# rajashree-srikanth/drone-sim-python

Measured on AMD Instinct MI355X. Metric: trajectory-optimisations/sec (6-seg poly, 50 wpts), higher is better.
Workload: dtype f64 residual/gradient + f32 MFMA J^T J

## Files before the change

drone-sim-python_amd/csrc/fit_basis.cpp:

```cpp
#include <cmath>
#include <cstring>

#include "fit_plan.h"

namespace {

double arr(int k, int n) {
  double a = 1;
  for (int i = n; i > n - k; --i) a *= i;
  return a;
}

struct Dense {
  int r, c;
  std::vector<double> a;
  Dense(int r_, int c_) : r(r_), c(c_), a((size_t)r_ * c_, 0.0) {}
  double &operator()(int i, int j) { return a[(size_t)i * c + j]; }
  double operator()(int i, int j) const { return a[(size_t)i * c + j]; }
};

Dense matmul(const Dense &A, const Dense &B, bool tA = false) {
  const int m = tA ? A.c : A.r, k = tA ? A.r : A.c, n = B.c;
  Dense C(m, n);
  for (int i = 0; i < m; ++i)
// ... 30 lines not shown
  for (int c = 0; c < n; ++c) {
    int piv = c;
    for (int r = c + 1; r < n; ++r)
      if (std::fabs(A(r, c)) > std::fabs(A(piv, c))) piv = r;
    if (A(piv, c) == 0.0) return false;
    for (int j = 0; j < n; ++j) {
      std::swap(A(c, j), A(piv, j));
      std::swap(I(c, j), I(piv, j));
    }
    const double ip = 1.0 / A(c, c);
    for (int j = 0; j < n; ++j) { A(c, j) *= ip; I(c, j) *= ip; }
    for (int r = 0; r < n; ++r) {
      if (r == c) continue;
      const double f = A(r, c);
      for (int j = 0; j < n; ++j) { A(r, j) -= f * A(c, j); I(r, j) -= f * I(c, j); }
    }
  }
  A = I;
  return true;
}

}

int fit_basis_build(d2d_fit_plan *pl) {
  const int S = pl->S, K = pl->K, nz = 8 * S, nk = 4 * (S + 1), nq = 4 * S;
  const double T = pl->duration / S;
  pl->T = T;
  pl->nq = nq;
  std::vector<int> seg(K);
  std::vector<double> tau(K);
  {
    std::vector<double> ends(S);
    double acc = 0;
    for (int s = 0; s < S; ++s) { acc += T; ends[s] = acc; }
    for (int k = 0; k < K; ++k) {
      const double step = pl->duration / (K - 1);
      const double t = (k == K - 1) ? pl->duration : k * step;
      int s = S - 1;
      for (int j = 0; j < S; ++j)
        if (ends[j] > t) { s = j; break; }
      seg[k] = s;
      tau[k] = t - s * T;
    }
  }
  pl->seg = seg;
  pl->tau = tau;
  std::vector<Dense> Phi;
  for (int d = 0; d < 3; ++d) {
    Dense P(K, nz);
    for (int k = 0; k < K; ++k)
      for (int p = d; p < 8; ++p) P(k, 8 * seg[k] + p) = arr(d, p) * std::pow(tau[k], p - d);
    Phi.push_back(P);
  }
  Dense M3(4, 4), M4(4, 4);
  for (int i = 0; i < 4; ++i) {
    for (int j = i; j < 4; ++j) M3(i, j) = arr(i, j) * std::pow(T, j - i);
    for (int j = 0; j < 4; ++j) M4(i, j) = arr(i, j + 4) * std::pow(T, j - i + 4);
  }
  if (!invert(M4)) { d2d_set_error("fit_basis_build: singular Hermite block"); return D2D_EINVAL; }
  Dense H(8, 8);
  for (int i = 0; i < 4; ++i) H(i, i) = 1.0 / arr(i, i);
  {
    Dense M1i(4, 4);
    for (int i = 0; i < 4; ++i) M1i(i, i) = 1.0 / arr(i, i);
    Dense t = matmul(matmul(M4, M3), M1i);
    for (int i = 0; i < 4; ++i)
      for (int j = 0; j < 4; ++j) { H(4 + i, j) = -t(i, j); H(4 + i, 4 + j) = M4(i, j); }
// ... 165 lines not shown
    A(k, k) = 1.0;
    for (int p = k; p < 8; ++p) {
      double c = 1.0;
      for (int i = 0; i < k; ++i) c = c * (p - i) / (i + 1);
      A(4 + k, p) = c;
    }
  }
  if (!invert(A)) { d2d_set_error("fit_basis_knots: singular Hermite block"); return D2D_EINVAL; }
  kn.Hb64.assign((size_t)K * KN_HB_STRIDE, 0.0);
  kn.Hb32.assign((size_t)K * 32, 0.f);
  for (int k = 0; k < K; ++k) {
    const double x = pl->tau[k] / T;
    const int s = pl->seg[k];
    for (int d = 0; d < 3; ++d)
      for (int m = 0; m < 8; ++m) {
        double v = 0.0;
        for (int p = d; p < 8; ++p) v += arr(d, p) * std::pow(x, p - d) * A(p, m);
        v /= std::pow(T, d);
        kn.Hb64[(size_t)k * KN_HB_STRIDE + 4 * m + d] = v;
        const bool fixed = (s == 0 && m < 2) || (s == S - 1 && m >= 4 && m < 6);
        kn.Hb32[(size_t)k * 32 + 4 * m + d] = fixed ? 0.f : (float)v;
      }
  }
  for (int s = 0; s <= S; ++s) kn.k0[s] = s < S ? pl->seg_k0[s] : K;
  for (int s = 0; s < S; ++s)
    if (pl->seg_Ks[s] == 0) kn.k0[s] = s + 1 < S ? pl->seg_k0[s + 1] : K;
  for (int s = S + 1; s <= D2D_FIT_MAX_S; ++s) kn.k0[s] = K;
  kn.Wseg.assign((size_t)S * 4 * 64, 0.f);
  for (int s = 0; s < S; ++s)
    for (int r = 0; r < 4; ++r)
      for (int l = 0; l < 64; ++l) {
        const int R = 4 * (l >> 4) + r, C = l & 15;
        const int aR = (R >> 2) & 1, aC = (C >> 2) & 1, mR = 4 * (R >> 3) + (R & 3), mC = 4 * (C >> 3) + (C & 3);
        if (aR != aC) continue;
        double v = 0.0;
        for (int k = kn.k0[s]; k < kn.k0[s + 1]; ++k) v += (double)kn.Hb32[(size_t)k * 32 + 4 * mR] * (double)kn.Hb32[(size_t)k * 32 + 4 * mC];
        kn.Wseg[((size_t)s * 4 + r) * 64 + l] = (float)v;
      }
  Dense L(nq, nq), Bm(nq, nq), Bi(nq, nq), Mu(nq, nq);
  for (int i = 0; i < nq; ++i)
    for (int j = 0; j < nq; ++j) L(i, j) = pl->Lw[(size_t)i * nq + j];
  std::vector<double> ds(nq);
  for (int i = 0; i < nq; ++i) ds[i] = dsc[freec[i] % 4];
  for (int j = 0; j < nq; ++j)
    for (int i = 0; i < nq; ++i) Bm(j, i) = L(i, j) / ds[i];
  Bi = Bm;
  if (!invert(Bi)) { d2d_set_error("fit_basis_knots: singular map"); return D2D_EINVAL; }
  Mu = matmul(Bm, Bm, true);
  Dense Mi = Mu;
  if (!invert(Mi)) { d2d_set_error("fit_basis_knots: singular metric"); return D2D_EINVAL; }
// ... 52 lines not shown
```

drone-sim-python_amd/csrc/fit_knot.hip:

```cpp
#include <cstdlib>
#include <vector>

#include "fit_phases.h"
#include "fit_plan.h"

#define KN_WPB_MAX 8
#define KN_LDS_BYTES (160 * 1024)
#define KN_N 48
#define KN_NE 56
#define KN_WV_KNOT 10
#define KN_US 10
#define KN_GTOL_SCALE 0.1
#define KN_SEG_MAX 11
#define KN_IMG_LS (KN_N + 4)

namespace {

#define LAUNDER_S(v) do { (v) = __builtin_amdgcn_readfirstlane(v); asm volatile("" : "+s"(v)); } while (0)

struct KnotGeom {
  int K, S, smax;
  int k0[D2D_FIT_MAX_S + 2];
};

struct KnotLds {
  int Hb64, Hb32, Wseg, Md32, Mi32, Mr32, Msc, wave0, wave_stride;
  int wv, sp, sfull, gfull, park, big, cf, cfp;
  int total;
};

inline int align16(int v) { return (v + 15) & ~15; }

KnotLds knot_lds_layout(int K, int wpb) {
  KnotLds L;
  int o = 0;
  L.Hb64 = o; o = align16(o + K * KN_HB_STRIDE * 8);
// ... 142 lines not shown
    for (int j = 0; j < 3; ++j) {
      const int s = s0 + j;
      int kb = kg.k0[s];
      n[j] = kg.k0[s + 1] - kg.k0[s];
      LAUNDER_S(kb); LAUNDER_S(n[j]);
#pragma unroll
      for (int i = 0; i < SEGMAX; ++i) {
        const int kk = kb + (i < n[j] ? i : (n[j] > 0 ? n[j] - 1 : 0));
        const float2 t = lds_get<float2>(lds + tab + kk * 128);
        const float2 cc = lds_get<float2>(lds + cfo + kk * 64);
        v[j][i] = fmaf(cc.y, t.y, cc.x * t.x);
      }
#pragma unroll
      for (int rr = 0; rr < 4; ++rr) acc[s][rr] = ww * Wseg[(s * 4 + rr) * 64 + lane];
    }
#pragma unroll
    for (int i = 0; i < SEGMAX; ++i)
#pragma unroll
      for (int j = 0; j < 3; ++j)
        if (i < n[j]) acc[s0 + j] = __builtin_amdgcn_mfma_f32_16x16x4f32(v[j][i], v[j][i], acc[s0 + j], 0, 0, 0);
  }
}

__device__ __forceinline__ void knot_mfma_so(const KnotGeom &kg, const unsigned char *lds, int hb32_off, int cf_off, int cfp_off,
                                             const float *Wseg, float ww, int lane, f32x4 (&acc)[D2D_FIT_MAX_S]) {
  LAUNDER(lane);
  const int c = lane & 15, rho = lane >> 4;
  const int m = 4 * (c >> 3) + (c & 3);
  const bool ay = ((c >> 2) & 1) != 0, row_y = (rho & 1) != 0, row_2 = rho >= 2;
  const int tab = hb32_off + 4 * m * 4;
  const int reco = cf_off + rho * 16 + (ay ? 8 : 0), rpo = cfp_off + (rho & 1) * 8 + (ay ? 4 : 0);
#pragma unroll
  for (int s = 0; s < D2D_FIT_MAX_S; ++s) {
#pragma unroll
    for (int rr = 0; rr < 4; ++rr) acc[s][rr] = ww * Wseg[(s * 4 + rr) * 64 + lane];
    int k1 = kg.k0[s + 1];
    int k = kg.k0[s];
    LAUNDER_S(k1); LAUNDER_S(k);
    if (k < k1) {
      f32x4 hb = lds_get<f32x4>(lds + tab + k * 128);
      float2 rec = lds_get<float2>(lds + reco + k * 64);
      float rp = lds_get<float>(lds + rpo + k * 16);
      for (; k < k1; ++k) {
        const int kn = k + 1 < k1 ? k + 1 : k;
        const f32x4 hbn = lds_get<f32x4>(lds + tab + kn * 128);
        const float2 recn = lds_get<float2>(lds + reco + kn * 64);
// ... 77 lines not shown
    float r = m0.x * s0.x;
    r = fmaf(m0.y, s0.y, r); r = fmaf(m0.z, s0.z, r); r = fmaf(m0.w, s0.w, r);
    r = fmaf(m1.x, s1.x, r); r = fmaf(m1.y, s1.y, r); r = fmaf(m1.z, s1.z, r); r = fmaf(m1.w, s1.w, r);
    r = fmaf(m2.x, s2.x, r); r = fmaf(m2.y, s2.y, r); r = fmaf(m2.z, s2.z, r); r = fmaf(m2.w, s2.w, r);
    return act ? r : 0.f;
  }
  int row_off;
  __device__ __forceinline__ void prepare(int l) { row_off = md32_off + (l < KN_N ? l : 0) * (KN_N * 4); }
  __device__ __forceinline__ f32x4 damp(int j0) const {
#ifdef KN_ABL_DAMP
    return f32x4{lam, lam, lam, lam};
#endif
    const float *mdrow = reinterpret_cast<const float *>(lds + row_off);
    return lam != 0.f ? lds_get<f32x4>(mdrow + j0) : f32x4{0.f, 0.f, 0.f, 0.f};
  }
};

}
template <> struct nd_is_banded<KnotMetric> { static constexpr bool value = true; };
static_assert(KN_N == 48 && D2D_FIT_MAX_S == 6, "nd_panel3_chunk0_zero<KnotMetric> rests on the 4 / 8 x 5 / 4 layout of the 48 free entries");
template <> struct nd_panel3_chunk0_zero<KnotMetric> { static constexpr bool value = true; };
namespace {

template <bool STAMPS, bool SEG9>
__global__ void __launch_bounds__(64 * KN_WPB_MAX)
fit_lm_knot_kernel(int B, KnotGeom kg, KnotLds L, d2d_fit_opts opts, int iter_cap, KnotDev T, const double *__restrict__ pk,
                   const double *__restrict__ prep, double *q_io, double *cost_io, double *g_io, double *lm, int32_t *flags,
                   int32_t *queue, const int32_t *__restrict__ order, int prio_at, double *u_io, unsigned long long *__restrict__ stamps,
                   float *dbg) {
  unsigned long long st_acc[8] = {0, 0, 0, 0, 0, 0, 0, 0}, st_last = 0;
#define KN_STAMP(i)                                                     \
  if (STAMPS) {                                                         \
    const unsigned long long t_ = __builtin_amdgcn_s_memtime();         \
    st_acc[i] += t_ - st_last;                                          \
    st_last = t_;                                                       \
  }
  extern __shared__ __attribute__((aligned(16))) unsigned char lds[];
  constexpr int N = KN_N;
  stage(lds + L.Hb64, T.Hb64, kg.K * KN_HB_STRIDE * 8);
  stage(lds + L.Hb32, T.Hb32, kg.K * 32 * 4);
  stage(lds + L.Wseg, T.Wseg, D2D_FIT_MAX_S * 4 * 64 * 4);
  stage(lds + L.Md32, T.Md32, N * N * 4);
  stage(lds + L.Mi32, T.Mi32, KN_NE * 28 * 4);
  stage(lds + L.Mr32, T.Mrow32, KN_NE * 12 * 4);
  stage(lds + L.Msc, T.msc, KN_NE * 8);
  __syncthreads();
  const double *Hb64 = reinterpret_cast<const double *>(lds + L.Hb64);
// ... 151 lines not shown
      const double xn = sqrt(fmax(uniform_d(wave_sum((double)dv * (double)mv)), 0.0));
      xub = xn * (1.0 + 1e-6);
      if (mp.first && V_mp_delta <= 0.0) V_mp_delta = xn > 0.0 ? 100.0 * xn : 100.0;
    }
    KN_STAMP(0)
    for (bool reenter = true; reenter;) {
      reenter = false;
      c = uniform_d(knot_phase1(kg.K, Hb64, sp, wv, seg_of_lane(), park, us, cf, cfp, so_rows, lane));
      KN_STAMP(1)
      bool fresh = true;
      if (!(fabs(c) <= 1.79e308)) { status = D2D_ST_NONFINITE; fresh = false; }
      int sub = 0, lp_it = 0, att = 0;
      V_alpha = 1.0;
      float dl = 0.f;
      bool fin = false, accept = false;
      while (status == D2D_ST_RUNNING || fresh) {
        bool do_solve = false, is_gn = false, do_trial = false;
        double solve_lam = 0.0;
        int isq_mode = 0;
        if (sub == 0) {
          if (fresh) {
            int p2_kb, p2_km, p2_ke;
            p2_ranges(p2_kb, p2_km, p2_ke);
            gi = knot_phase2(kg, Hb64, us, p2_kb, p2_km, p2_ke, ea, ekd, act, lane);
            KN_STAMP(2)
            fresh = false;
            if (status != D2D_ST_RUNNING) break;
            f32x4 acc[D2D_FIT_MAX_S];
            const float ww = (float)(sp[PR_WWP] * sp[PR_WWP]);
            const int wbase = L.wave0 + wave * L.wave_stride;
            if (so_rows) knot_mfma_so(kg, lds, L.Hb32, wbase + L.cf, wbase + L.cfp, Wseg, ww, lane, acc);
            else if (SEG9) knot_mfma<9>(kg, lds, L.Hb32, wbase + L.cf, Wseg, ww, lane, acc);
            else knot_mfma<KN_SEG_MAX>(kg, lds, L.Hb32, wbase + L.cf, Wseg, ww, lane, acc);
            nev += so_rows ? 3 : 2;
            wave_lds_sync();
            KN_STAMP(3)
            knot_blocks_to_image(acc, big, lane);
            image_put_rhs<N>(big, lane, gi);
            wave_lds_sync();
            image_row<N>(big, lane, hrow);
            hdiag = image_diag<N>(big, lane);
            wave_lds_sync();
            if (STAMPS && dbg != nullptr && iters == 0 && act) {
              float *d = dbg + (size_t)b * (N * N + 4 * N) + lane * N;
#pragma unroll
              for (int m = 0; m < N / 2; ++m) { d[2 * m] = hrow[m].x; d[2 * m + 1] = hrow[m].y; }
              dbg[(size_t)b * (N * N + 4 * N) + N * N + lane] = (float)gi;
              dbg[(size_t)b * (N * N + 4 * N) + N * N + N + lane] = (float)ui;
            }
            gnrm = -1.0;
            KN_STAMP(4)
          }
          if (iters >= iter_cap || iters >= opts.max_iter) break;
          if (iters >= prio_at) __builtin_amdgcn_s_setprio(2);
// ... 284 lines not shown
  pl->kn.wpb = 0;
  if (pl->S != 6 || pl->nq != 24 || pl->K > 64) return D2D_OK;
  if (int rc = fit_basis_knots(pl)) return rc;
  for (int s2 = 0; s2 < pl->S; ++s2)
    if (pl->kn.k0[s2 + 1] - pl->kn.k0[s2] > KN_SEG_MAX) return D2D_OK;
  int wpb = 0;
  for (int w = KN_WPB_MAX; w >= 4; --w)
    if (knot_lds_layout(pl->K, w).total <= KN_LDS_BYTES) { wpb = w; break; }
  if (wpb == 0) return D2D_OK;
  auto &kn = pl->kn;
  int rc = upload(&kn.d_Hb64, kn.Hb64);
  if (!rc) rc = upload(&kn.d_Hb32, kn.Hb32);
  if (!rc) rc = upload(&kn.d_Wseg, kn.Wseg);
  if (!rc) rc = upload(&kn.d_Md32, kn.Md32);
  if (!rc) rc = upload(&kn.d_Mrow32, kn.Mrow32);
  if (!rc) rc = upload(&kn.d_Mi32, kn.Mi32);
  if (!rc) rc = upload(&kn.d_Bq, kn.Bq);
  if (!rc) rc = upload(&kn.d_BiT, kn.BiT);
  if (!rc) rc = upload(&kn.d_Binv, kn.Binv);
  if (!rc) rc = upload(&kn.d_Minv, kn.Minv);
  if (!rc) rc = upload(&kn.d_Pu, kn.Pu);
  if (!rc) rc = upload(&kn.d_msc, kn.msc);
  if (rc) return rc;
  (void)hipFuncSetAttribute(reinterpret_cast<const void *>(&fit_lm_knot_kernel<false, false>), hipFuncAttributeMaxDynamicSharedMemorySize, KN_LDS_BYTES);
  (void)hipFuncSetAttribute(reinterpret_cast<const void *>(&fit_lm_knot_kernel<true, false>), hipFuncAttributeMaxDynamicSharedMemorySize, KN_LDS_BYTES);
  (void)hipFuncSetAttribute(reinterpret_cast<const void *>(&fit_lm_knot_kernel<false, true>), hipFuncAttributeMaxDynamicSharedMemorySize, KN_LDS_BYTES);
  (void)hipFuncSetAttribute(reinterpret_cast<const void *>(&fit_lm_knot_kernel<true, true>), hipFuncAttributeMaxDynamicSharedMemorySize, KN_LDS_BYTES);
  kn.wpb = wpb;
  return D2D_OK;
}

void fit_knot_plan_free(d2d_fit_plan *pl) {
  auto &kn = pl->kn;
  void *p[] = {kn.d_Hb64, kn.d_Hb32, kn.d_Wseg, kn.d_Md32, kn.d_Mrow32, kn.d_Mi32, kn.d_Bq, kn.d_BiT, kn.d_Binv, kn.d_Minv, kn.d_Pu, kn.d_msc, kn.d_u};
  for (void *q : p)
    if (q) hipFree(q);
  kn.d_Hb64 = kn.d_Bq = kn.d_BiT = kn.d_Binv = kn.d_Minv = kn.d_Pu = kn.d_msc = kn.d_u = nullptr;
  kn.d_Hb32 = kn.d_Wseg = kn.d_Md32 = kn.d_Mrow32 = kn.d_Mi32 = nullptr;
  kn.wpb = 0;
}

int fit_knot_ensure(d2d_fit_plan *pl, int cap_B) {
  auto &kn = pl->kn;
  if (kn.wpb == 0) return D2D_OK;
  if (kn.d_u) { hipFree(kn.d_u); kn.d_u = nullptr; }
  D2D_CHECK_HIP(hipMalloc(&kn.d_u, (size_t)cap_B * 64 * sizeof(double)));
  D2D_CHECK_HIP(hipMemset(kn.d_u, 0, (size_t)cap_B * 64 * sizeof(double)));
  return D2D_OK;
}

int fit_knot_launch(d2d_ctx *ctx, d2d_fit_plan *pl, int B, double *q, const d2d_fit_opts &o, int iter_cap, const int32_t *order, int prio_at) {
  auto &kn = pl->kn;
  KnotGeom kg;
  kg.K = pl->K; kg.S = pl->S; kg.smax = 0;
  for (int s = 0; s <= D2D_FIT_MAX_S + 1; ++s) kg.k0[s] = kn.k0[s < D2D_FIT_MAX_S + 2 ? s : D2D_FIT_MAX_S + 1];
  for (int j = 0; j < pl->S; ++j)
    if (kn.k0[j + 1] - kn.k0[j] > kg.smax) kg.smax = kn.k0[j + 1] - kn.k0[j];
  const KnotLds L = knot_lds_layout(pl->K, kn.wpb);
  KnotDev T{kn.d_Hb64, kn.d_Bq, kn.d_BiT, kn.d_Binv, kn.d_Minv, kn.d_Pu, kn.d_msc, kn.d_Hb32, kn.d_Wseg, kn.d_Md32, kn.d_Mrow32, kn.d_Mi32};
  static const bool want_stamps = getenv("D2D_LM_STAMPS") != nullptr || getenv("D2D_KNOT_DEBUG") != nullptr;
  unsigned long long *stamps = want_stamps ? reinterpret_cast<unsigned long long *>(ctx->stats_dev + 8) : nullptr;
  if (want_stamps) D2D_CHECK_HIP(hipMemsetAsync(stamps, 0, 8 * sizeof(unsigned long long), ctx->stream));
  const int blocks = B < pl->n_cu ? B : pl->n_cu;
  int32_t *queue = ctx->counter_dev + 8;
  float *dbg = nullptr;
  if (getenv("D2D_KNOT_DEBUG")) D2D_CHECK_HIP(hipMalloc(&dbg, (size_t)B * (KN_N * KN_N + 4 * KN_N) * sizeof(float)));
#define KN_LAUNCH(ST, S9)                                                                                                                  \
  hipLaunchKernelGGL((fit_lm_knot_kernel<ST, S9>), dim3(blocks), dim3(64 * kn.wpb), L.total, ctx->stream, B, kg, L, o, iter_cap, T, pl->d_pk, \
                     pl->d_prep, q, pl->d_cost, pl->d_g, pl->d_lm, pl->d_flags, queue, order, prio_at, kn.d_u, stamps, dbg)
  const bool seg9 = kg.smax <= 9;
  if (want_stamps) { if (seg9) KN_LAUNCH(true, true); else KN_LAUNCH(true, false); }
  else { if (seg9) KN_LAUNCH(false, true); else KN_LAUNCH(false, false); }
#undef KN_LAUNCH
  D2D_LAUNCH_CHECK();
  if (dbg) {
    std::vector<float> h((size_t)B * (KN_N * KN_N + 4 * KN_N));
    D2D_CHECK_HIP(hipMemcpyAsync(h.data(), dbg, h.size() * sizeof(float), hipMemcpyDeviceToHost, ctx->stream));
    D2D_CHECK_HIP(hipStreamSynchronize(ctx->stream));
    if (FILE *f = fopen(getenv("D2D_KNOT_DEBUG"), "wb")) { fwrite(h.data(), sizeof(float), h.size(), f); fclose(f); }
    hipFree(dbg);
  }
  if (want_stamps) {
    unsigned long long h[8];
    D2D_CHECK_HIP(hipMemcpyAsync(h, stamps, sizeof(h), hipMemcpyDeviceToHost, ctx->stream));
    D2D_CHECK_HIP(hipStreamSynchronize(ctx->stream));
    static const char *nm[7] = {"io/loop", "phase1", "phase2", "mfma", "image+gnrm", "solve", "judge"};
    double tot = 0;
    for (int i = 0; i < 7; ++i) tot += (double)h[i];
    fprintf(stderr, "[fit_lm_knot stamps] wave-cycles (s_memtime ticks), B=%d iter_cap=%d:", B, iter_cap);
    for (int i = 0; i < 7; ++i) fprintf(stderr, " %s=%.1f%%", nm[i], 100.0 * (double)h[i] / tot);
    fprintf(stderr, " total=%.3e\n", tot);
  }
  return D2D_OK;
}
```

drone-sim-python_amd/csrc/fit_plan.h:

```cpp
#pragma once
#include <vector>

#include "common.h"

enum { FL_STATUS = 0, FL_ITERS = 1, FL_NEED = 2, FL_NEVAL = 3 };
#define LM_STRIDE 8

#define KN_HB_STRIDE 34
struct KnotTables {
  int NE = 0, NV = 0;
  int k0[D2D_FIT_MAX_S + 2] = {0};
  std::vector<double> Hb64, Bq, BiT, Binv, Minv, Mrow, Pu, msc;
  std::vector<float> Hb32, Wseg, Md32, Mrow32, Mi32;
  double *d_Hb64 = nullptr, *d_Bq = nullptr, *d_BiT = nullptr, *d_Binv = nullptr, *d_Minv = nullptr, *d_Pu = nullptr, *d_msc = nullptr;
  float *d_Hb32 = nullptr, *d_Wseg = nullptr, *d_Md32 = nullptr, *d_Mrow32 = nullptr, *d_Mi32 = nullptr;
  double *d_u = nullptr;
  int wpb = 0;
};

struct d2d_fit_plan {
  int device;
  int S, K, nq;
  double duration, T;
  double wref[3];
// ... 39 lines not shown
  int32_t *d_ring = nullptr;
  int ring_cap = 0;
  int gorder_R = 0, gsweeps_R = 0;
  int n_group = 1, nds = 0;
  const double *prep_valid_for = nullptr;
  bool g32_lds = true;
  int wpb_eval = 8, wpb_step = 8, wpb_lm = 0;
  bool use_lm = false;
  bool use_long = false;
  bool split_ok = true;
  int n_cu = 256;
  int kernel_req = D2D_FIT_KERNEL_AUTO, long_tables = -1;
  int it_done = 0, active_B = 0;
  const double *solve_q = nullptr;
  int solve_kernel = -1;
  int last_slice = 0, last_running = -1;
  d2d_fit_opts last_opts = {};
  bool prof_on = false;
  std::vector<hipEvent_t> prof_ev;
  std::vector<int> prof_kind;
};

int fit_basis_build(d2d_fit_plan *pl);
int fit_basis_segments(d2d_fit_plan *pl);
int fit_basis_knots(d2d_fit_plan *pl);
int fit_knot_plan_init(d2d_fit_plan *pl);
void fit_knot_plan_free(d2d_fit_plan *pl);
int fit_knot_ensure(d2d_fit_plan *pl, int cap_B);
int fit_knot_launch(d2d_ctx *ctx, d2d_fit_plan *pl, int B, double *q, const d2d_fit_opts &o, int iter_cap, const int32_t *order, int prio_at);
```

drone-sim-python_amd/d2dhip/__init__.py:

```python
import ctypes as C
import os

import numpy as np

_HERE = os.path.dirname(os.path.abspath(__file__))
LIB_PATH = os.environ.get('D2D_LIB') or os.path.join(os.path.dirname(_HERE), 'lib', 'libd2dhip.so')

SCEN_STRIDE = 80
MAX_OBS = 16
MAX_MOV, MOV_MAX_KNOT = 8, 32
MAX_VIA = 16
(SC_X0, SC_Y0, SC_PSI0, SC_X1, SC_Y1, SC_PSI1, SC_VREF, SC_VSP, SC_KV, SC_KPHI, SC_KOBS, SC_S,
 SC_WWP, SC_WX, SC_WY, SC_GOLEFT, SC_O0X, SC_O0Y, SC_O0R, SC_O1X, SC_O1Y, SC_O1R, SC_WBND,
 SC_PHIMAX, SC_VMIN, SC_VMAX, SC_KCOL, SC_RCOL, SC_SCOL, SC_PMASK, SC_OKIND, SC_BANKMAX, SC_OEXT) = range(33)
SC_XMIN, SC_XMAX, SC_YMIN, SC_YMAX = range(SC_OEXT + 3 * (MAX_OBS - 2), SC_OEXT + 3 * (MAX_OBS - 2) + 4)


def obs_col(i):
    return SC_O0X + 3 * i if i < 2 else SC_OEXT + 3 * (i - 2)


TRAJ_MAX_SEG, TRAJ_SEG_STRIDE = 8, 20
TRAJ_STRIDE = 4 + TRAJ_MAX_SEG * TRAJ_SEG_STRIDE
TRAJ_LINE, TRAJ_CIRCLE, TRAJ_SLALOM, TRAJ_POLY = 1, 2, 3, 4
# ... 139 lines not shown
    'd2d_nlp_solve_groups': (C.c_int, [_P, C.c_int, C.c_int, C.c_int, C.c_double, _P, C.POINTER(NlpOpts), C.c_int, C.c_double] + [_P] * 9),
    'd2d_nlp_solve_groups_wind': (C.c_int, [_P, C.c_int, C.c_int, C.c_int, C.c_double, _P, C.POINTER(NlpOpts), C.c_int, C.c_double] + [_P] * 9
                                  + [C.POINTER(WindFieldC), _P]),
    'd2d_nlp_solve_groups_pairs': (C.c_int, [_P, C.c_int, C.c_int, C.c_int, C.c_double, _P, C.POINTER(NlpOpts), C.c_int, C.c_double] + [_P] * 9
                                   + [C.POINTER(WindFieldC), _P]),
    'd2d_nlp_solve_model': (C.c_int, [_P, C.c_int, C.c_int, C.c_double, _P, C.POINTER(NlpOpts), C.POINTER(NlpModel)] + [_P] * 7),
    'd2d_mov_sample': (C.c_int, [_P, C.c_int, C.c_int, C.c_double, _P, C.POINTER(MovingObstaclesC), _P]),
    'd2d_nlp_solve_moving': (C.c_int, [_P, C.c_int, C.c_int, C.c_double, _P, C.POINTER(NlpOpts)] + [_P] * 7
                             + [C.POINTER(WindFieldC), _P, C.POINTER(MovingObstaclesC), _P]),
    'd2d_nlp_solve_groups_moving': (C.c_int, [_P, C.c_int, C.c_int, C.c_int, C.c_double, _P, C.POINTER(NlpOpts), C.c_int, C.c_double] + [_P] * 9
                                    + [C.POINTER(WindFieldC), _P, C.POINTER(MovingObstaclesC), _P]),
    'd2d_nlp_solve_via': (C.c_int, [_P, C.c_int, C.c_int, C.c_double, _P, C.POINTER(NlpOpts)] + [_P] * 7
                          + [C.POINTER(WindFieldC), _P, C.POINTER(MovingObstaclesC), _P, C.POINTER(ViaPointsC), _P]),
    'd2d_nlp_solve_groups_via': (C.c_int, [_P, C.c_int, C.c_int, C.c_int, C.c_double, _P, C.POINTER(NlpOpts), C.c_int, C.c_double] + [_P] * 9
                                 + [C.POINTER(WindFieldC), _P, C.POINTER(MovingObstaclesC), _P, C.POINTER(ViaPointsC), _P]),
    'd2d_flight_audit_workspace': (C.c_int64, [C.POINTER(AuditParams), C.c_int]),
    'd2d_flight_audit': (C.c_int, [_P, C.POINTER(AuditParams)] + [_P] * 6 + [C.POINTER(MovingObstaclesC), _P, _P, C.POINTER(AuditOut)]),
    'd2d_fit_plan_create': (C.c_int, [_P, C.c_int, C.c_int, C.c_double, _P, C.POINTER(_P)]),
    'd2d_fit_plan_create_ex': (C.c_int, [_P, C.c_int, C.c_int, C.c_double, _P, C.POINTER(FitPlanOpts), C.POINTER(_P)]),
    'd2d_fit_opts_default': (C.c_int, [C.POINTER(FitOpts)]),
    'd2d_fit_plan_destroy': (C.c_int, [_P]),
    'd2d_fit_plan_get': (C.c_int, [_P] * 6),
    'd2d_fit_plan_kernel': (C.c_int, [_P]),
    'd2d_fit_init': (C.c_int, [_P, _P, C.c_int, _P, _P]),
    'd2d_fit_project': (C.c_int, [_P, _P, C.c_int, _P, _P, _P]),
    'd2d_fit_eval': (C.c_int, [_P, _P, C.c_int, _P, _P, _P, _P, _P]),
    'd2d_fit_rows': (C.c_int, [_P, _P, C.c_int, _P, _P, _P, _P]),
    'd2d_fit_jtj': (C.c_int, [_P, _P, C.c_int, _P]),
    'd2d_fit_solve': (C.c_int, [_P, _P, C.c_int, _P, _P, C.POINTER(FitOpts), _P, _P, _P, _P]),
    'd2d_fit_begin': (C.c_int, [_P, _P, C.c_int]),
    'd2d_fit_iterate': (C.c_int, [_P, _P, C.c_int, _P, _P, C.POINTER(FitOpts), C.c_int, C.POINTER(C.c_int32)]),
    'd2d_fit_finish': (C.c_int, [_P, _P, C.c_int, _P, _P, _P, _P, _P, _P]),
    'd2d_fit_plan_set_order': (C.c_int, [_P, _P, C.c_int, _P]),
    'd2d_fit_plan_set_handout_prior': (C.c_int, [_P, _P, _P]),
    'd2d_fit_plan_get_order': (C.c_int, [_P, _P, C.c_int, _P]),
    'd2d_fit_plan_set_group_order': (C.c_int, [_P, _P, C.c_int, C.c_int]),
    'd2d_fit_group_report': (C.c_int, [_P, _P, C.c_int, _P, _P]),
    'd2d_fit_plan_set_groups': (C.c_int, [_P, C.c_int]),
    'd2d_fit_solve_groups': (C.c_int, [_P, _P, C.c_int, _P, _P, C.POINTER(FitOpts), C.c_int, C.c_int, C.c_double, _P,
                                       C.POINTER(C.c_int32), _P]),
    'd2d_fit_profile': (C.c_int, [_P, C.c_int]),
    'd2d_fit_profile_read': (C.c_int, [_P, _P]),
    'd2d_fit_coeffs': (C.c_int, [_P, _P, C.c_int, _P, _P, _P]),
    'd2d_fit_sample': (C.c_int, [_P, _P, C.c_int, _P, _P, _P, _P]),
}
EXPORTS = tuple(_SIGS)

_lib = None


def load():
    global _lib
    if _lib is not None:
        return _lib
    if not os.path.exists(LIB_PATH):
        raise D2DError(f'{LIB_PATH} not found: build it with __graft_entry__.build() '
                       f'(make -C drone-sim-python_amd/csrc); there is no CPU fallback')
    lib = C.CDLL(LIB_PATH)
    for name, (res, args) in _SIGS.items():
        fn = getattr(lib, name)
        fn.restype, fn.argtypes = res, args
    _lib = lib
    return lib


def _check(rc):
    if rc != 0:
        raise D2DError(f'libd2dhip error {rc}: {load().d2d_last_error().decode()}')


def _torch():
    import torch
    if not torch.cuda.is_available():
        raise D2DError('no HIP device visible to PyTorch-ROCm; the d2d engine has no CPU fallback')
    return torch


_ABSENT = object()


def _ptr(t):
    return None if t is None else C.c_void_p(t.data_ptr())


def _hptr(a):
    return None if a is None else a.ctypes.data_as(C.c_void_p)


def _wind_c(ctx, wind):
    if isinstance(wind, WindFieldC):
        return wind
# ... 671 lines not shown
```

include/d2d.h:

```cpp
#ifndef D2D_H
#define D2D_H

#include <stdint.h>

#ifdef __cplusplus
extern "C" {
#endif

#define D2D_VERSION 118

#define D2D_OK 0
#define D2D_EINVAL (-1)
#define D2D_EHIP (-2)
#define D2D_ENOMEM (-3)
#define D2D_ESTATE (-4)

typedef struct d2d_ctx d2d_ctx;
typedef struct d2d_fit_plan d2d_fit_plan;

int d2d_version(void);
const char *d2d_last_error(void);

int d2d_ctx_create(int device, void *stream, d2d_ctx **out);
int d2d_ctx_destroy(d2d_ctx *ctx);
int d2d_ctx_sync(d2d_ctx *ctx);

typedef struct d2d_comm d2d_comm;
#define D2D_COMM_ID_BYTES 128
int d2d_comm_available(void);
int d2d_comm_unique_id(void *id_out);
int d2d_comm_create(d2d_ctx *ctx, const void *id, int rank, int world, d2d_comm **out);
int d2d_comm_destroy(d2d_comm *comm);
// ... 187 lines not shown
  int32_t gs_ls;
  int32_t gs_ls_s0;
  double gs_ls_r0;
  int32_t gs_prio_at;
  int32_t gs_pairs;
} d2d_fit_opts;
enum { D2D_HANDOUT_INDEX = 0, D2D_HANDOUT_PREDICTED = 1 };
#define D2D_LM_PRIO_AT 48
int d2d_fit_opts_default(d2d_fit_opts *o);

int d2d_fit_plan_create(d2d_ctx *ctx, int S, int K, double duration, const double *wref,
                        d2d_fit_plan **out);
#define D2D_FIT_KERNEL_AUTO (-1)
typedef struct {
  int32_t kernel;
  int32_t long_tables;
  int32_t reserved[2];
} d2d_fit_plan_opts;
int d2d_fit_plan_create_ex(d2d_ctx *ctx, int S, int K, double duration, const double *wref, const d2d_fit_plan_opts *popts,
                           d2d_fit_plan **out);
int d2d_fit_plan_destroy(d2d_fit_plan *plan);
enum { D2D_FIT_KERNEL_SPLIT = 0, D2D_FIT_KERNEL_FUSED = 1, D2D_FIT_KERNEL_LONG = 2, D2D_FIT_KERNEL_KNOT = 3 };
int d2d_fit_plan_kernel(const d2d_fit_plan *plan);

int d2d_fit_plan_get(const d2d_fit_plan *plan, double *G, double *Gp, double *Z, double *Zp,
                     double *Pinit);

int d2d_fit_init(d2d_ctx *ctx, const d2d_fit_plan *plan, int B, const double *scen, double *q);

int d2d_fit_project(d2d_ctx *ctx, const d2d_fit_plan *plan, int B, const double *scen, const double *xy,
                    double *q);

int d2d_fit_eval(d2d_ctx *ctx, const d2d_fit_plan *plan, int B, const double *scen,
                 const double *q, double *cost, double *g, float *H);

int d2d_fit_rows(d2d_ctx *ctx, d2d_fit_plan *plan, int B, const double *scen, const double *q, double *cost, double *g);
int d2d_fit_jtj(d2d_ctx *ctx, d2d_fit_plan *plan, int B, float *H);

int d2d_fit_solve(d2d_ctx *ctx, const d2d_fit_plan *plan, int B, const double *scen, double *q,
                  const d2d_fit_opts *opts, double *cost, int32_t *iters, int32_t *status,
                  double *stats);

int d2d_fit_begin(d2d_ctx *ctx, d2d_fit_plan *plan, int B);
int d2d_fit_iterate(d2d_ctx *ctx, d2d_fit_plan *plan, int B, const double *scen, double *q,
                    const d2d_fit_opts *opts, int n_iters, int32_t *n_running);
int d2d_fit_finish(d2d_ctx *ctx, d2d_fit_plan *plan, int B, const double *scen, const double *q,
// ... 146 lines not shown
```

Measured before the change: 1.720 million.

## Fuse f64 gradient phase into MFMA J^T J loop with software-pipelined LDS reads

Adds a fused kernel variant that interleaves the f64 phase-2 gradient accumulation with the f32 MFMA J^T J accumulation. It uses a fixed per-segment sample floor so the first SEGMIN samples run unmasked with a multi-stage operand pipeline and explicit schedule barriers. The variant is picked at launch when S is 6 and every segment has at least 8 samples, which holds for 50 waypoints. This is meant to hide LDS and global load latency behind the MFMAs and drop the separate phase-2 pass. In exchange it adds template instantiations and register pressure, and it recomputes the segment start indices directly from the sample segments.

```diff
diff --git a/drone-sim-python_amd/csrc/fit_basis.cpp b/drone-sim-python_amd/csrc/fit_basis.cpp
--- a/drone-sim-python_amd/csrc/fit_basis.cpp
+++ b/drone-sim-python_amd/csrc/fit_basis.cpp
@@ -76,27 +76,54 @@
 
 }
 
+void fit_basis_sample_segments(int S, int K, double duration, std::vector<int> &seg, std::vector<double> &tau) {
+  const double T = duration / S;
+  seg.assign(K, 0);
+  tau.assign(K, 0.0);
+  std::vector<double> ends(S);
+  double acc = 0;
+  for (int s = 0; s < S; ++s) { acc += T; ends[s] = acc; }
+  for (int k = 0; k < K; ++k) {
+    const double step = duration / (K - 1);
+    const double t = (k == K - 1) ? duration : k * step;
+    int s = S - 1;
+    for (int j = 0; j < S; ++j)
+      if (ends[j] > t) { s = j; break; }
+    seg[k] = s;
+    tau[k] = t - s * T;
+  }
+}
+
+void fit_knot_first_samples(const std::vector<int> &seg, int S, int *k0) {
+  const int K = (int)seg.size();
+  for (int s = 0; s <= D2D_FIT_MAX_S; ++s) k0[s] = K;
+  for (int k = K - 1; k >= 0; --k) k0[seg[k]] = k;
+  for (int s = S - 1; s >= 0; --s) {
+    bool any = false;
+    for (int k = 0; k < K && !any; ++k) any = seg[k] == s;
+    if (!any) k0[s] = k0[s + 1];
+  }
+}
+
+void fit_knot_seg_range(const int *k0, int S, int *smin, int *smax) {
+  int lo = S > 0 ? k0[1] - k0[0] : 0, hi = lo;
+  for (int s = 1; s < S; ++s) {
+    const int n = k0[s + 1] - k0[s];
+    lo = n < lo ? n : lo;
+    hi = n > hi ? n : hi;
+  }
+  if (smin) *smin = lo;
+  if (smax) *smax = hi;
+}
+
 int fit_basis_build(d2d_fit_plan *pl) {
   const int S = pl->S, K = pl->K, nz = 8 * S, nk = 4 * (S + 1), nq = 4 * S;
   const double T = pl->duration / S;
   pl->T = T;
   pl->nq = nq;
-  std::vector<int> seg(K);
-  std::vector<double> tau(K);
-  {
-    std::vector<double> ends(S);
-    double acc = 0;
-    for (int s = 0; s < S; ++s) { acc += T; ends[s] = acc; }
-    for (int k = 0; k < K; ++k) {
-      const double step = pl->duration / (K - 1);
-      const double t = (k == K - 1) ? pl->duration : k * step;
-      int s = S - 1;
-      for (int j = 0; j < S; ++j)
-        if (ends[j] > t) { s = j; break; }
-      seg[k] = s;
-      tau[k] = t - s * T;
-    }
-  }
+  std::vector<int> seg;
+  std::vector<double> tau;
+  fit_basis_sample_segments(S, K, pl->duration, seg, tau);
   pl->seg = seg;
   pl->tau = tau;
   std::vector<Dense> Phi;
@@ -308,10 +335,7 @@
         kn.Hb32[(size_t)k * 32 + 4 * m + d] = fixed ? 0.f : (float)v;
       }
   }
-  for (int s = 0; s <= S; ++s) kn.k0[s] = s < S ? pl->seg_k0[s] : K;
-  for (int s = 0; s < S; ++s)
-    if (pl->seg_Ks[s] == 0) kn.k0[s] = s + 1 < S ? pl->seg_k0[s + 1] : K;
-  for (int s = S + 1; s <= D2D_FIT_MAX_S; ++s) kn.k0[s] = K;
+  fit_knot_first_samples(pl->seg, S, kn.k0);
   kn.Wseg.assign((size_t)S * 4 * 64, 0.f);
   for (int s = 0; s < S; ++s)
     for (int r = 0; r < 4; ++r)
diff --git a/drone-sim-python_amd/csrc/fit_knot.hip b/drone-sim-python_amd/csrc/fit_knot.hip
--- a/drone-sim-python_amd/csrc/fit_knot.hip
+++ b/drone-sim-python_amd/csrc/fit_knot.hip
@@ -12,6 +12,8 @@
 #define KN_US 10
 #define KN_GTOL_SCALE 0.1
 #define KN_SEG_MAX 11
+#define KN_FUSED_DEPTH 6
+#define KN_SEG_FLOOR 8
 #define KN_IMG_LS (KN_N + 4)
 
 namespace {
@@ -200,6 +202,105 @@
   }
 }
 
+template <int SEGMAX, int SEGMIN>
+__device__ __forceinline__ double knot_eval_fused(const KnotGeom &kg, const unsigned char *lds, const double *Hb64, const double *us,
+                                                  int kb, int km, int ke, int a, int kd, bool live, int hb32_off, int cf_off,
+                                                  const float *Wseg, float ww, int lane, f32x4 (&acc)[D2D_FIT_MAX_S]) {
+  typedef double __attribute__((ext_vector_type(2), may_alias)) f64x2a;
+  constexpr int SLOTS = (SEGMAX + 2) / 3 * 3;
+  static_assert(SEGMIN > 0 && SEGMIN <= SEGMAX && SEGMIN % 3 != 0, "a masked sample follows the floor in every half");
+  static_assert(D2D_FIT_MAX_S == 6, "two halves of three segments");
+  LAUNDER(lane);
+  LAUNDER(kb);
+  const int c = lane & 15, r = lane >> 4;
+  const int m = 4 * (c >> 3) + (c & 3), ax = (c >> 2) & 1;
+  const int tab = hb32_off + (4 * m + (r < 2 ? 1 : 0)) * 4;
+  const int cfo = cf_off + r * 16 + ax * 8;
+  double a0 = 0.0, a1 = 0.0, a2 = 0.0;
+#pragma unroll
+  for (int half = 0; half < 2; ++half) {
+    const int s0 = 3 * half;
+    const int k0 = half ? km : kb, k1 = half ? ke : km;
+    const int n = live ? k1 - k0 : 0;
+    const bool some = n > 0;
+    const int k0r = some ? k0 : 0;
+    const double *hb = Hb64 + (size_t)k0r * KN_HB_STRIDE + 4 * ((half ? 0 : 4) + kd);
+    const double *uk = us + k0r * KN_US + 4 * a;
+    const double b0 = a0, b1 = a1, b2 = a2;
+    constexpr int NQ = 3 * SEGMIN, TAIL = SEGMAX - SEGMIN, DEPTH = KN_FUSED_DEPTH;
+    static_assert(SEGMIN >= 4, "the operand pipeline is two rows deep");
+    const unsigned char *tp[3], *cp[3];
+    float2 rt[DEPTH], rc[DEPTH], rtt[3][TAIL > 0 ? TAIL : 1], rct[3][TAIL > 0 ? TAIL : 1];
+    float vq[2], vt[3][TAIL > 0 ? TAIL : 1];
+    int ns[3];
+#pragma unroll
+    for (int j = 0; j < 3; ++j) {
+      const int s = s0 + j;
+      int sb = kg.k0[s];
+      ns[j] = kg.k0[s + 1] - kg.k0[s];
+      LAUNDER_S(sb); LAUNDER_S(ns[j]);
+      tp[j] = lds + tab + sb * 128; cp[j] = lds + cfo + sb * 64;
+#pragma unroll
+      for (int i = 0; i < DEPTH / 3; ++i) { rt[3 * i + j] = lds_get<float2>(tp[j] + i * 128); rc[3 * i + j] = lds_get<float2>(cp[j] + i * 64); }
+#pragma unroll
+      for (int rr = 0; rr < 4; ++rr) acc[s][rr] = ww * Wseg[(s * 4 + rr) * 64 + lane];
+    }
+    vq[0] = fmaf(rc[0].y, rt[0].y, rc[0].x * rt[0].x);
+    __builtin_amdgcn_sched_barrier(0);
+    constexpr int LAG = 3, STEP = (NQ - 1 - LAG) / (SLOTS - 1), NBUF = LAG / (STEP > 0 ? STEP : 1) + 1;
+    static_assert(STEP >= 1, "every sample of the half finds its two k-steps");
+    f64x2a h01[NBUF], u01[NBUF];
+    double h2[NBUF], u2[NBUF];
+    auto p2_read = [&](int idx, int i) {
+      if (idx < SEGMIN) {
+        h01[i] = *reinterpret_cast<const f64x2a *>(hb + idx * KN_HB_STRIDE); u01[i] = *reinterpret_cast<const f64x2a *>(uk + idx * KN_US);
+        h2[i] = hb[idx * KN_HB_STRIDE + 2]; u2[i] = uk[idx * KN_US + 2];
+      } else {
+        const bool in = idx < n;
+        const int o = in ? idx : 0;
+        const f64x2a hr = *reinterpret_cast<const f64x2a *>(hb + o * KN_HB_STRIDE), ur = *reinterpret_cast<const f64x2a *>(uk + o * KN_US);
+        const double h2r = hb[o * KN_HB_STRIDE + 2], u2r = uk[o * KN_US + 2];
+        h01[i] = in ? hr : f64x2a{0.0, 0.0}; u01[i] = in ? ur : f64x2a{0.0, 0.0};
+        h2[i] = in ? h2r : 0.0; u2[i] = in ? u2r : 0.0;
+      }
+    };
+    auto p2_fma = [&](int idx, int i) {
+      if (idx == SEGMIN) { a0 = some ? a0 : b0; a1 = some ? a1 : b1; a2 = some ? a2 : b2; }
+      a0 = fma(h01[i].x, u01[i].x, a0);
+      a1 = fma(h01[i].y, u01[i].y, a1);
+      a2 = fma(h2[i], u2[i], a2);
+      LAUNDER(a0); LAUNDER(a1); LAUNDER(a2);
+    };
+#pragma unroll
+    for (int q = 0; q < NQ; ++q) {
+      const int i = q / 3, j = q % 3;
+      acc[s0 + j] = __builtin_amdgcn_mfma_f32_16x16x4f32(vq[q & 1], vq[q & 1], acc[s0 + j], 0, 0, 0);
+      if (q + DEPTH < NQ) {
+        rt[q % DEPTH] = lds_get<float2>(tp[j] + (i + DEPTH / 3) * 128); rc[q % DEPTH] = lds_get<float2>(cp[j] + (i + DEPTH / 3) * 64);
+      } else if (q + 6 < NQ + 3 && q + 6 >= NQ) {
+#pragma unroll
+        for (int t = 0; t < TAIL; ++t) {
+          const int kk = SEGMIN + t < ns[j] ? SEGMIN + t : ns[j] - 1;
+          rtt[j][t] = lds_get<float2>(tp[j] + kk * 128); rct[j][t] = lds_get<float2>(cp[j] + kk * 64);
+        }
+      } else if (q + 3 >= NQ) {
+#pragma unroll
+        for (int t = 0; t < TAIL; ++t) vt[j][t] = fmaf(rct[j][t].y, rtt[j][t].y, rct[j][t].x * rtt[j][t].x);
+      }
+      if (q % STEP == 0 && q / STEP < SLOTS) p2_read(q / STEP, (q / STEP) % NBUF);
+      if (q >= LAG && (q - LAG) % STEP == 0 && (q - LAG) / STEP < SLOTS) p2_fma((q - LAG) / STEP, ((q - LAG) / STEP) % NBUF);
+      if (q + 1 < NQ) vq[(q + 1) & 1] = fmaf(rc[(q + 1) % DEPTH].y, rt[(q + 1) % DEPTH].y, rc[(q + 1) % DEPTH].x * rt[(q + 1) % DEPTH].x);
+      __builtin_amdgcn_sched_barrier(0);
+    }
+#pragma unroll
+    for (int t = 0; t < TAIL; ++t)
+#pragma unroll
+      for (int j = 0; j < 3; ++j)
+        if (SEGMIN + t < ns[j]) acc[s0 + j] = __builtin_amdgcn_mfma_f32_16x16x4f32(vt[j][t], vt[j][t], acc[s0 + j], 0, 0, 0);
+  }
+  return (a0 + a1) + a2;
+}
+
 __device__ __forceinline__ void knot_mfma_so(const KnotGeom &kg, const unsigned char *lds, int hb32_off, int cf_off, int cfp_off,
                                              const float *Wseg, float ww, int lane, f32x4 (&acc)[D2D_FIT_MAX_S]) {
   LAUNDER(lane);
@@ -323,7 +424,7 @@
 template <> struct nd_panel3_chunk0_zero<KnotMetric> { static constexpr bool value = true; };
 namespace {
 
-template <bool STAMPS, bool SEG9>
+template <bool STAMPS, bool SEG9, int SEGMIN>
 __global__ void __launch_bounds__(64 * KN_WPB_MAX)
 fit_lm_knot_kernel(int B, KnotGeom kg, KnotLds L, d2d_fit_opts opts, int iter_cap, KnotDev T, const double *__restrict__ pk,
                    const double *__restrict__ prep, double *q_io, double *cost_io, double *g_io, double *lm, int32_t *flags,
@@ -521,14 +622,18 @@
           if (fresh) {
             int p2_kb, p2_km, p2_ke;
             p2_ranges(p2_kb, p2_km, p2_ke);
-            gi = knot_phase2(kg, Hb64, us, p2_kb, p2_km, p2_ke, ea, ekd, act, lane);
+            f32x4 acc[D2D_FIT_MAX_S];
+            const float ww = (float)(sp[PR_WWP] * sp[PR_WWP]);
+            const int wbase = L.wave0 + wave * L.wave_stride;
+            const bool fused = SEGMIN > 0 && !so_rows && status == D2D_ST_RUNNING;
+            if (!fused) gi = knot_phase2(kg, Hb64, us, p2_kb, p2_km, p2_ke, ea, ekd, act, lane);
             KN_STAMP(2)
             fresh = false;
             if (status != D2D_ST_RUNNING) break;
-            f32x4 acc[D2D_FIT_MAX_S];
-            const float ww = (float)(sp[PR_WWP] * sp[PR_WWP]);
-            const int wbase = L.wave0 + wave * L.wave_stride;
             if (so_rows) knot_mfma_so(kg, lds, L.Hb32, wbase + L.cf, wbase + L.cfp, Wseg, ww, lane, acc);
+            else if constexpr (SEGMIN > 0)
+              gi = knot_eval_fused<(SEG9 ? 9 : KN_SEG_MAX), SEGMIN>(kg, lds, Hb64, us, p2_kb, p2_km, p2_ke, ea, ekd, act, L.Hb32, wbase + L.cf,
+                                                                    Wseg, ww, lane, acc);
             else if (SEG9) knot_mfma<9>(kg, lds, L.Hb32, wbase + L.cf, Wseg, ww, lane, acc);
             else knot_mfma<KN_SEG_MAX>(kg, lds, L.Hb32, wbase + L.cf, Wseg, ww, lane, acc);
             nev += so_rows ? 3 : 2;
@@ -859,10 +964,11 @@
   if (!rc) rc = upload(&kn.d_Pu, kn.Pu);
   if (!rc) rc = upload(&kn.d_msc, kn.msc);
   if (rc) return rc;
-  (void)hipFuncSetAttribute(reinterpret_cast<const void *>(&fit_lm_knot_kernel<false, false>), hipFuncAttributeMaxDynamicSharedMemorySize, KN_LDS_BYTES);
-  (void)hipFuncSetAttribute(reinterpret_cast<const void *>(&fit_lm_knot_kernel<true, false>), hipFuncAttributeMaxDynamicSharedMemorySize, KN_LDS_BYTES);
-  (void)hipFuncSetAttribute(reinterpret_cast<const void *>(&fit_lm_knot_kernel<false, true>), hipFuncAttributeMaxDynamicSharedMemorySize, KN_LDS_BYTES);
-  (void)hipFuncSetAttribute(reinterpret_cast<const void *>(&fit_lm_knot_kernel<true, true>), hipFuncAttributeMaxDynamicSharedMemorySize, KN_LDS_BYTES);
+#define KN_ATTR(ST, S9, SM) \
+  (void)hipFuncSetAttribute(reinterpret_cast<const void *>(&fit_lm_knot_kernel<ST, S9, SM>), hipFuncAttributeMaxDynamicSharedMemorySize, KN_LDS_BYTES)
+  KN_ATTR(false, false, 0); KN_ATTR(true, false, 0); KN_ATTR(false, true, 0); KN_ATTR(true, true, 0);
+  KN_ATTR(false, false, KN_SEG_FLOOR); KN_ATTR(true, false, KN_SEG_FLOOR); KN_ATTR(false, true, KN_SEG_FLOOR); KN_ATTR(true, true, KN_SEG_FLOOR);
+#undef KN_ATTR
   kn.wpb = wpb;
   return D2D_OK;
 }
@@ -886,13 +992,29 @@
   return D2D_OK;
 }
 
+static int knot_seg_floor(int S, int smin) { return S == D2D_FIT_MAX_S && smin >= KN_SEG_FLOOR ? KN_SEG_FLOOR : 0; }
+
+int d2d_fit_knot_segments(int S, int K, double duration, int32_t *k0, int32_t *seg_min, int32_t *seg_max, int32_t *seg_floor) {
+  if (S < 1 || S > D2D_FIT_MAX_S || K < 2 || !(duration > 0.0)) { d2d_set_error("d2d_fit_knot_segments: S in 1 .. %d, K >= 2, duration > 0", D2D_FIT_MAX_S); return D2D_EINVAL; }
+  std::vector<int> seg;
+  std::vector<double> tau;
+  fit_basis_sample_segments(S, K, duration, seg, tau);
+  int first[D2D_FIT_MAX_S + 2] = {0}, smin = 0, smax = 0;
+  fit_knot_first_samples(seg, S, first);
+  fit_knot_seg_range(first, S, &smin, &smax);
+  if (k0) for (int s = 0; s <= S; ++s) k0[s] = first[s];
+  if (seg_min) *seg_min = smin;
+  if (seg_max) *seg_max = smax;
+  if (seg_floor) *seg_floor = knot_seg_floor(S, smin);
+  return D2D_OK;
+}
+
 int fit_knot_launch(d2d_ctx *ctx, d2d_fit_plan *pl, int B, double *q, const d2d_fit_opts &o, int iter_cap, const int32_t *order, int prio_at) {
   auto &kn = pl->kn;
   KnotGeom kg;
   kg.K = pl->K; kg.S = pl->S; kg.smax = 0;
   for (int s = 0; s <= D2D_FIT_MAX_S + 1; ++s) kg.k0[s] = kn.k0[s < D2D_FIT_MAX_S + 2 ? s : D2D_FIT_MAX_S + 1];
-  for (int j = 0; j < pl->S; ++j)
-    if (kn.k0[j + 1] - kn.k0[j] > kg.smax) kg.smax = kn.k0[j + 1] - kn.k0[j];
+  fit_knot_seg_range(kn.k0, pl->S, nullptr, &kg.smax);
   const KnotLds L = knot_lds_layout(pl->K, kn.wpb);
   KnotDev T{kn.d_Hb64, kn.d_Bq, kn.d_BiT, kn.d_Binv, kn.d_Minv, kn.d_Pu, kn.d_msc, kn.d_Hb32, kn.d_Wseg, kn.d_Md32, kn.d_Mrow32, kn.d_Mi32};
   static const bool want_stamps = getenv("D2D_LM_STAMPS") != nullptr || getenv("D2D_KNOT_DEBUG") != nullptr;
@@ -902,12 +1024,21 @@
   int32_t *queue = ctx->counter_dev + 8;
   float *dbg = nullptr;
   if (getenv("D2D_KNOT_DEBUG")) D2D_CHECK_HIP(hipMalloc(&dbg, (size_t)B * (KN_N * KN_N + 4 * KN_N) * sizeof(float)));
-#define KN_LAUNCH(ST, S9)                                                                                                                  \
-  hipLaunchKernelGGL((fit_lm_knot_kernel<ST, S9>), dim3(blocks), dim3(64 * kn.wpb), L.total, ctx->stream, B, kg, L, o, iter_cap, T, pl->d_pk, \
+#define KN_LAUNCH(ST, S9, SM)                                                                                                                  \
+  hipLaunchKernelGGL((fit_lm_knot_kernel<ST, S9, SM>), dim3(blocks), dim3(64 * kn.wpb), L.total, ctx->stream, B, kg, L, o, iter_cap, T, pl->d_pk, \
                      pl->d_prep, q, pl->d_cost, pl->d_g, pl->d_lm, pl->d_flags, queue, order, prio_at, kn.d_u, stamps, dbg)
-  const bool seg9 = kg.smax <= 9;
-  if (want_stamps) { if (seg9) KN_LAUNCH(true, true); else KN_LAUNCH(true, false); }
-  else { if (seg9) KN_LAUNCH(false, true); else KN_LAUNCH(false, false); }
+#define KN_LAUNCH_SEG(ST)                                                                     \
+  do {                                                                                        \
+    if (floor8) { if (seg9) KN_LAUNCH(ST, true, KN_SEG_FLOOR); else KN_LAUNCH(ST, false, KN_SEG_FLOOR); } \
+    else { if (seg9) KN_LAUNCH(ST, true, 0); else KN_LAUNCH(ST, false, 0); }                  \
+  } while (0)
+  const char *ablate = getenv("D2D_FIT_ABLATE");
+  const bool force_generic = ablate != nullptr && (atoi(ablate) & 64) != 0;
+  int smin = 0, smax = 0;
+  fit_knot_seg_range(kn.k0, pl->S, &smin, &smax);
+  const bool seg9 = smax <= 9, floor8 = knot_seg_floor(pl->S, smin) == KN_SEG_FLOOR && !force_generic;
+  if (want_stamps) KN_LAUNCH_SEG(true); else KN_LAUNCH_SEG(false);
+#undef KN_LAUNCH_SEG
 #undef KN_LAUNCH
   D2D_LAUNCH_CHECK();
   if (dbg) {
diff --git a/drone-sim-python_amd/csrc/fit_plan.h b/drone-sim-python_amd/csrc/fit_plan.h
--- a/drone-sim-python_amd/csrc/fit_plan.h
+++ b/drone-sim-python_amd/csrc/fit_plan.h
@@ -85,6 +85,9 @@
 };
 
 int fit_basis_build(d2d_fit_plan *pl);
+void fit_basis_sample_segments(int S, int K, double duration, std::vector<int> &seg, std::vector<double> &tau);
+void fit_knot_first_samples(const std::vector<int> &seg, int S, int *k0);
+void fit_knot_seg_range(const int *k0, int S, int *smin, int *smax);
 int fit_basis_segments(d2d_fit_plan *pl);
 int fit_basis_knots(d2d_fit_plan *pl);
 int fit_knot_plan_init(d2d_fit_plan *pl);
diff --git a/drone-sim-python_amd/d2dhip/__init__.py b/drone-sim-python_amd/d2dhip/__init__.py
--- a/drone-sim-python_amd/d2dhip/__init__.py
+++ b/drone-sim-python_amd/d2dhip/__init__.py
@@ -185,6 +185,7 @@
     'd2d_fit_plan_destroy': (C.c_int, [_P]),
     'd2d_fit_plan_get': (C.c_int, [_P] * 6),
     'd2d_fit_plan_kernel': (C.c_int, [_P]),
+    'd2d_fit_knot_segments': (C.c_int, [C.c_int, C.c_int, C.c_double, _P, _P, _P, _P]),
     'd2d_fit_init': (C.c_int, [_P, _P, C.c_int, _P, _P]),
     'd2d_fit_project': (C.c_int, [_P, _P, C.c_int, _P, _P, _P]),
     'd2d_fit_eval': (C.c_int, [_P, _P, C.c_int, _P, _P, _P, _P, _P]),
@@ -230,6 +231,15 @@
 def _check(rc):
     if rc != 0:
         raise D2DError(f'libd2dhip error {rc}: {load().d2d_last_error().decode()}')
+
+
+def knot_segments(S, K, duration):
+    import numpy as np
+    k0 = np.zeros(S + 1, dtype=np.int32)
+    out = (C.c_int32 * 3)()
+    p = [C.cast(C.byref(out, 4 * i), C.c_void_p) for i in range(3)]
+    _check(load().d2d_fit_knot_segments(S, K, float(duration), _hptr(k0), *p))
+    return k0, int(out[0]), int(out[1]), int(out[2])
 
 
 def _torch():
diff --git a/include/d2d.h b/include/d2d.h
--- a/include/d2d.h
+++ b/include/d2d.h
@@ -7,7 +7,7 @@
 extern "C" {
 #endif
 
-#define D2D_VERSION 118
+#define D2D_VERSION 119
 
 #define D2D_OK 0
 #define D2D_EINVAL (-1)
@@ -241,6 +241,7 @@
 int d2d_fit_plan_destroy(d2d_fit_plan *plan);
 enum { D2D_FIT_KERNEL_SPLIT = 0, D2D_FIT_KERNEL_FUSED = 1, D2D_FIT_KERNEL_LONG = 2, D2D_FIT_KERNEL_KNOT = 3 };
 int d2d_fit_plan_kernel(const d2d_fit_plan *plan);
+int d2d_fit_knot_segments(int S, int K, double duration, int32_t *k0, int32_t *seg_min, int32_t *seg_max, int32_t *seg_floor);
 
 int d2d_fit_plan_get(const d2d_fit_plan *plan, double *G, double *Gp, double *Z, double *Zp,
                      double *Pinit);
```

Measured after the change: 1.792 million, median of 6. +4.2%, better.
